# kartikmadhira1/YA_VO

Measured on AMD Instinct MI355X. Metric: frames/sec (detect+describe+match+PnP) on 1241×376 KITTI stereo; RMSE vs CPU ref, higher is better.
Workload: dtype u8

## Files before the change

ya_vo_amd/csrc/yavo_kernels.hip:

```cpp
#include <hip/hip_runtime.h>
#include <stdint.h>
#include <stdlib.h>
#include <string.h>

#include <algorithm>

#include "yavo_xlane.h"
#include "yavo_internal.h"


namespace yavo {

__device__ __forceinline__ int lane_id() { return (int)(threadIdx.x & 63); }

__device__ __forceinline__ int wave_incl_scan(int v) {
    v += __builtin_amdgcn_update_dpp(0, v, 0x111, 0xf, 0xf, false);
    v += __builtin_amdgcn_update_dpp(0, v, 0x112, 0xf, 0xf, false);
    v += __builtin_amdgcn_update_dpp(0, v, 0x114, 0xf, 0xf, false);
    v += __builtin_amdgcn_update_dpp(0, v, 0x118, 0xf, 0xf, false);
    v += __builtin_amdgcn_update_dpp(0, v, 0x142, 0xa, 0xf, false);
    v += __builtin_amdgcn_update_dpp(0, v, 0x143, 0xc, 0xf, false);
    return v;
}

// ... 929 lines not shown
                const int g = item & 3, kd = (item >> 2) * 64 + ln;
                const int k = (kd & 31) * G + (kd >> 5);
                const bool act = (kd >> 5) < G && k < nb;
                const uint32_t e = s_list[act ? k : nb - 1];
                const int i = (int)(e >> 16), row = r0 + (int)(e & 31u), col = (int)((e >> 5) & 2047u);
                const int id = (act && g == 0) ? src[i].z : 0;
                const int la = (row - rb) * LS + col;
                const int2* lo = loff + 64 * g;
                uint32_t w[2] = {0u, 0u};
#pragma unroll 1
                for (int c = 7; c >= 0; --c) {
                    const int2* oc = lo + 8 * c;
                    uint32_t acc = w[c >> 2];
#pragma unroll
                    for (int j = 7; j >= 0; --j) {
                        const int2 o = oc[j];
                        const uint32_t p1 = s_band[la + o.x], p2 = s_band[la + o.y];
                        acc = __builtin_amdgcn_alignbit(acc, p2 - p1, 31);
                    }
                    if (c >= 4) w[1] = acc;
                    else w[0] = acc;
                }
                if (act) {
                    reinterpret_cast<uint2*>(d_base + i)[g] = make_uint2(w[0], w[1]);
                    uint8_t* r = rec_b + (int64_t)i * 48;
                    if (g == 0) {
                        reinterpret_cast<int32_t*>(r)[0] = row;
                        reinterpret_cast<int32_t*>(r)[1] = col;
                        reinterpret_cast<int32_t*>(r)[2] = id;
                        r[12] = 0;
                    }
                    r[13 + 8 * g] = (uint8_t)w[0];
                    *reinterpret_cast<uint16_t*>(r + 14 + 8 * g) = (uint16_t)(w[0] >> 8);
                    *reinterpret_cast<uint32_t*>(r + 16 + 8 * g) = (w[0] >> 24) | (w[1] << 8);
                    r[20 + 8 * g] = (uint8_t)(w[1] >> 24);
                    if (g == 3) {
                        r[45] = 0;
                        *reinterpret_cast<uint16_t*>(r + 46) = 0;
                    }
                }
                asm volatile("" ::"v"(id));
            }
        }
        BP_MARK(1);
        __builtin_amdgcn_fence(__ATOMIC_RELEASE, "workgroup", "local");
        __builtin_amdgcn_s_barrier();
        __builtin_amdgcn_fence(__ATOMIC_ACQUIRE, "workgroup", "local");
        lb = __builtin_amdgcn_readfirstlane(s_next[0]);
        klo = __builtin_amdgcn_readfirstlane(s_next[1]);
        nbk = __builtin_amdgcn_readfirstlane(s_next[2]);
        BP_MARK(2);
    }
    BP_STORE();
}

__global__ void brief_loff_kernel(const int8_t* __restrict__ offsets, int LS, int2* __restrict__ loff) {
    const int t = threadIdx.x;
    const int8_t* o = offsets + 4 * t;
    loff[t] = make_int2((int)o[0] * LS + (int)o[1], (int)o[2] * LS + (int)o[3]);
}

void launch_brief(const uint8_t* blur, int n_images, int H, int W, const int8_t* offsets, const int32_t* kp_src,
                  const int32_t* kp_band, const int32_t* band_off, int max_kp, yv_keypoint* keypoints, Desc* desc,
                  int32_t* loff, bool new_loff, int32_t* heads, int max_workers, hipStream_t s) {
    const int total = ((H + BR_BAND - 1) / BR_BAND) * n_images;
    dim3 grid(std::max(1, std::min(max_workers, total)));
    const size_t lds = brief_lds_bytes(W);
    int2* lo = reinterpret_cast<int2*>(loff);
    if (new_loff) hipLaunchKernelGGL(brief_loff_kernel, dim3(1), dim3(256), 0, s, offsets, brief_lds_stride(W), lo);
    hipLaunchKernelGGL(brief_kernel, grid, dim3(BR_NT), lds, s, blur, H, W, kp_src, kp_band, band_off, max_kp,
                       keypoints, desc, lo, heads, total);
}

__global__ void pack_desc_kernel(const yv_keypoint* __restrict__ keypoints, const int32_t* __restrict__ kp_count,
                                 int max_kp, Desc* __restrict__ desc) {
    const int slot = blockIdx.y;
    const int i = blockIdx.x * blockDim.x + threadIdx.x;
    if (i >= kp_count[slot] || i >= max_kp) return;
    const uint8_t* rec = reinterpret_cast<const uint8_t*>(keypoints + (int64_t)slot * max_kp + i);
    Desc d;
#pragma unroll
    for (int q = 0; q < 8; ++q) {
        d.w[q] = (uint32_t)rec[13 + 4 * q] | ((uint32_t)rec[14 + 4 * q] << 8) | ((uint32_t)rec[15 + 4 * q] << 16) |
                 ((uint32_t)rec[16 + 4 * q] << 24);
    }
    desc[(int64_t)slot * max_kp + i] = d;
}

void launch_pack_desc(const yv_keypoint* keypoints, const int32_t* kp_count, int n_slots, int max_kp, Desc* desc,
                      hipStream_t s) {
    dim3 grid((max_kp + 255) / 256, n_slots);
    hipLaunchKernelGGL(pack_desc_kernel, grid, dim3(256), 0, s, keypoints, kp_count, max_kp, desc);
}

typedef int mm_v4i __attribute__((ext_vector_type(4)));
constexpr int MM_QT = 8;
constexpr int MM_QB = 4 * MM_QT * 16;
constexpr int MM_TC = 128;
constexpr int MM_ROW = 17;

__device__ __forceinline__ uint32_t expand_pm1(uint32_t nib) {
    const uint32_t spread = (nib * 0x00204081u) & 0x01010101u;
    return ~(spread * 0xFEu);
}

__device__ __forceinline__ uint4 expand16_pm1(uint32_t bits) {
    return make_uint4(expand_pm1(bits & 0xF), expand_pm1((bits >> 4) & 0xF), expand_pm1((bits >> 8) & 0xF),
                      expand_pm1((bits >> 12) & 0xF));
}

__device__ __forceinline__ int desc_popcount(const Desc& d) {
    int c = 0;
#pragma unroll
    for (int w = 0; w < 8; ++w) c += __popc(d.w[w]);
    return c;
}

__device__ __forceinline__ void top2_push2_i32(int& m1, int& m2, int x, int y) {
    const int hi = max(x, y), lo = min(x, y);
    m2 = max(min(m1, hi), max(m2, lo));
    m1 = max(m1, hi);
}

__device__ __forceinline__ void top2_merge_i32(int& m1, int& m2, int o1, int o2) {
    m2 = max(min(m1, o1), max(m2, o2));
    m1 = max(m1, o1);
}

__device__ __forceinline__ uint32_t mm_decode_key(int v) {
    const int dot = v >> 16;
    const uint32_t d = (uint32_t)((256 - dot) >> 1);
    const uint32_t jj = 0xFFFFu - ((uint32_t)v & 0xFFFFu);
    return (d << 16) | jj;
}

template <bool TOP2>
__device__ __forceinline__ void match_body(const Desc* __restrict__ desc, const int32_t* __restrict__ kp_count,
                                           const int32_t* __restrict__ pairs, int max_kp,
                                           uint32_t* __restrict__ match_key, uint32_t* __restrict__ match_key2) {
    __shared__ uint4 s_t[2][MM_TC * MM_ROW];
    const int pair = blockIdx.y;
    const int qi = pairs[2 * pair], ti = pairs[2 * pair + 1];
    const int nq = kp_count[qi], nt = kp_count[ti];
    const int q0 = blockIdx.x * MM_QB;
    if (q0 >= nq) return;
    const int tid = threadIdx.x, wave = tid >> 6, lane = tid & 63;
    const int col = lane & 15, g = lane >> 4;
    const Desc* qd = desc + (int64_t)qi * max_kp;
    const uint32_t* tw = reinterpret_cast<const uint32_t*>(desc + (int64_t)ti * max_kp);

    mm_v4i A[MM_QT][4];
#pragma unroll
    for (int qt = 0; qt < MM_QT; ++qt) {
        const int q = q0 + 16 * MM_QT * wave + 16 * qt + col;
        const Desc d = qd[q < nq ? q : 0];
#pragma unroll
        for (int s = 0; s < 4; ++s) {
            const uint32_t hi_mask = 0u - (uint32_t)(g >> 1);
            const uint32_t w = d.w[2 * s] ^ ((d.w[2 * s] ^ d.w[2 * s + 1]) & hi_mask);
            const uint32_t bits = (w >> (16 * (g & 1))) & 0xFFFFu;
            const uint4 e = expand16_pm1(bits);
            A[qt][s] = mm_v4i{(int)e.x, (int)e.y, (int)e.z, (int)e.w};
        }
    }
    int best[MM_QT][4];
#pragma unroll
    for (int qt = 0; qt < MM_QT; ++qt)
#pragma unroll
        for (int r = 0; r < 4; ++r) best[qt][r] = INT_MIN;
    int best2[TOP2 ? MM_QT : 1][4];
    if constexpr (TOP2) {
#pragma unroll
        for (int qt = 0; qt < MM_QT; ++qt)
#pragma unroll
            for (int r = 0; r < 4; ++r) best2[qt][r] = INT_MIN;
    }

    constexpr int kF = MM_TC * 16 / 256;
    uint32_t pre[kF];
    auto fetch = [&](int t0) {
#pragma unroll
        for (int k = 0; k < kF; ++k) {
            const int idx = tid + 256 * k, tt = idx >> 4, u = idx & 15;
            const int t = t0 + tt;
            pre[k] = t < nt ? tw[(int64_t)t * 8 + (u >> 1)] : 0u;
        }
    };
    auto store = [&](int buf) {
#pragma unroll
        for (int k = 0; k < kF; ++k) {
            const int idx = tid + 256 * k, tt = idx >> 4, u = idx & 15;
            const uint32_t bits = (pre[k] >> (16 * (u & 1))) & 0xFFFFu;
            s_t[buf][tt * MM_ROW + u] = expand16_pm1(bits);
        }
    };
    if (nt > 0) {
        fetch(0);
        store(0);
    }
    int buf = 0;
    for (int t0 = 0; t0 < nt; t0 += MM_TC) {
        const bool more = t0 + MM_TC < nt;
        if (more) fetch(t0 + MM_TC);
        __syncthreads();
#pragma unroll
        for (int tt0 = 0; tt0 < MM_TC; tt0 += 32) {
            if (t0 + tt0 >= nt) break;
            mm_v4i Ba[4], Bb[4];
#pragma unroll
            for (int s = 0; s < 4; ++s) {
                const uint4 va = s_t[buf][(tt0 + col) * MM_ROW + 4 * s + g];
                const uint4 vb = s_t[buf][(tt0 + 16 + col) * MM_ROW + 4 * s + g];
                Ba[s] = mm_v4i{(int)va.x, (int)va.y, (int)va.z, (int)va.w};
                Bb[s] = mm_v4i{(int)vb.x, (int)vb.y, (int)vb.z, (int)vb.w};
            }
            const int ja = t0 + tt0 + col, jb = ja + 16;
            {
                const int bias_a = ja < nt ? 0xFFFF - ja : -(1 << 30);
                const int bias_b = jb < nt ? 0xFFFF - jb : -(1 << 30);
#pragma unroll
                for (int qt = 0; qt < MM_QT; qt += 2) {
                    mm_v4i a0 = {0, 0, 0, 0}, b0 = {0, 0, 0, 0}, a1 = {0, 0, 0, 0}, b1 = {0, 0, 0, 0};
#pragma unroll
                    for (int s = 0; s < 4; ++s) {
                        a0 = __builtin_amdgcn_mfma_i32_16x16x64_i8(A[qt][s], Ba[s], a0, 0, 0, 0);
                        b0 = __builtin_amdgcn_mfma_i32_16x16x64_i8(A[qt][s], Bb[s], b0, 0, 0, 0);
                        a1 = __builtin_amdgcn_mfma_i32_16x16x64_i8(A[qt + 1][s], Ba[s], a1, 0, 0, 0);
                        b1 = __builtin_amdgcn_mfma_i32_16x16x64_i8(A[qt + 1][s], Bb[s], b1, 0, 0, 0);
                    }
#pragma unroll
                    for (int r = 0; r < 4; ++r) {
                        if constexpr (TOP2) {
                            top2_push2_i32(best[qt][r], best2[qt][r], (int)(((uint32_t)a0[r] << 16) + (uint32_t)bias_a),
                                           (int)(((uint32_t)b0[r] << 16) + (uint32_t)bias_b));
                            top2_push2_i32(best[qt + 1][r], best2[qt + 1][r],
                                           (int)(((uint32_t)a1[r] << 16) + (uint32_t)bias_a),
                                           (int)(((uint32_t)b1[r] << 16) + (uint32_t)bias_b));
                            continue;
                        }
                        best[qt][r] = max(best[qt][r], max((int)(((uint32_t)a0[r] << 16) + (uint32_t)bias_a),
                                                           (int)(((uint32_t)b0[r] << 16) + (uint32_t)bias_b)));
                        best[qt + 1][r] = max(best[qt + 1][r],
                                              max((int)(((uint32_t)a1[r] << 16) + (uint32_t)bias_a),
                                                  (int)(((uint32_t)b1[r] << 16) + (uint32_t)bias_b)));
                    }
                }
            }
        }
        if (more) {
            store(buf ^ 1);
            buf ^= 1;
        }
    }
#pragma unroll
    for (int qt = 0; qt < MM_QT; ++qt) {
#pragma unroll
        for (int r = 0; r < 4; ++r) {
            int v = best[qt][r];
            const int q = q0 + 16 * MM_QT * wave + 16 * qt + 4 * g + r;
            if constexpr (TOP2) {
                int v2 = best2[qt][r];
                top2_merge_i32(v, v2, xl::xor_row_i32<8>(v), xl::xor_row_i32<8>(v2));
                top2_merge_i32(v, v2, xl::xor_row_i32<4>(v), xl::xor_row_i32<4>(v2));
                top2_merge_i32(v, v2, xl::xor_row_i32<2>(v), xl::xor_row_i32<2>(v2));
                top2_merge_i32(v, v2, xl::xor_row_i32<1>(v), xl::xor_row_i32<1>(v2));
                if (col == r && q < nq) {
                    match_key[(int64_t)pair * max_kp + q] = v > -(1 << 29) ? mm_decode_key(v) : 0xFFFFFFFFu;
                    match_key2[(int64_t)pair * max_kp + q] = v2 > -(1 << 29) ? mm_decode_key(v2) : 0xFFFFFFFFu;
                }
                continue;
            }
            v = max(v, xl::xor_row_i32<8>(v));
            v = max(v, xl::xor_row_i32<4>(v));
            v = max(v, xl::xor_row_i32<2>(v));
            v = max(v, xl::xor_row_i32<1>(v));
            if (col == r && q < nq) {
                uint32_t key = 0xFFFFFFFFu;
                if (v != INT_MIN) {
                    const int dot = v >> 16;
                    const uint32_t d = (uint32_t)((256 - dot) >> 1);
                    const uint32_t jj = 0xFFFFu - ((uint32_t)v & 0xFFFFu);
                    key = (d << 16) | jj;
                }
                match_key[(int64_t)pair * max_kp + q] = key;
            }
        }
    }
}

__global__ __launch_bounds__(256) void match_kernel(const Desc* __restrict__ desc, const int32_t* __restrict__ kp_count,
                                                    const int32_t* __restrict__ pairs, int max_kp,
                                                    uint32_t* __restrict__ match_key) {
    match_body<false>(desc, kp_count, pairs, max_kp, match_key, nullptr);
}

__global__ __launch_bounds__(256) void match_top2_kernel(const Desc* __restrict__ desc,
                                                         const int32_t* __restrict__ kp_count,
                                                         const int32_t* __restrict__ pairs, int max_kp,
                                                         uint32_t* __restrict__ match_key,
                                                         uint32_t* __restrict__ match_key2) {
    match_body<true>(desc, kp_count, pairs, max_kp, match_key, match_key2);
}

constexpr int MF_TC = 128;
constexpr int MF_ROW = 9;
constexpr int MF2_QT = 4, MF2_WPE = 3;

__device__ __forceinline__ uint4 expand32_fp4(uint32_t w) {
    constexpr uint32_t kBit1 = 0x22222222u;
    return make_uint4((w << 1) & kBit1, w & kBit1, (w >> 1) & kBit1, (w >> 2) & kBit1);
}

typedef int mf_v8i __attribute__((ext_vector_type(8)));
typedef float mf_v16f __attribute__((ext_vector_type(16)));

__device__ __forceinline__ mf_v16f mfma_fp4_32(const mm_v4i& a, const mm_v4i& b, const mf_v16f& c) {
    const mf_v8i a8 = __builtin_shufflevector(a, a, 0, 1, 2, 3, -1, -1, -1, -1);
    const mf_v8i b8 = __builtin_shufflevector(b, b, 0, 1, 2, 3, -1, -1, -1, -1);
    return __builtin_amdgcn_mfma_scale_f32_32x32x64_f8f6f4(a8, b8, c, 4, 4, 0, 133, 0, 133);
}

__device__ __forceinline__ uint32_t max16_u32(uint32_t best, const mf_v16f& a) {
    auto u = [&](int i) { return __float_as_uint(a[i]); };
    const uint32_t m0 = max(u(0), max(u(1), u(2))), m1 = max(u(3), max(u(4), u(5)));
    const uint32_t m2 = max(u(6), max(u(7), u(8))), m3 = max(u(9), max(u(10), u(11)));
    const uint32_t m4 = max(u(12), max(u(13), u(14)));
    const uint32_t m5 = max(m0, max(m1, m2)), m6 = max(m3, max(m4, u(15)));
    return max(best, max(m5, m6));
}

__device__ __forceinline__ uint32_t umed3_pos(uint32_t a, uint32_t b, uint32_t c) {
    return __float_as_uint(__builtin_amdgcn_fmed3f(__uint_as_float(a), __uint_as_float(b), __uint_as_float(c)));
}

__device__ __forceinline__ void top2_merge3(uint32_t h0, uint32_t l0, uint32_t h1, uint32_t l1, uint32_t h2,
                                            uint32_t l2, uint32_t& m1, uint32_t& m2) {
    m1 = max(h0, max(h1, h2));
    m2 = max(umed3_pos(h0, h1, h2), max(l0, max(l1, l2)));
}

__device__ __forceinline__ void top2_16_u32(uint32_t& m1, uint32_t& m2, const mf_v16f& a) {
    auto u = [&](int i) { return __float_as_uint(a[i]); };
    uint32_t h[5], l[5];
#pragma unroll
    for (int k = 0; k < 5; ++k) {
        h[k] = max(u(3 * k), max(u(3 * k + 1), u(3 * k + 2)));
        l[k] = umed3_pos(u(3 * k), u(3 * k + 1), u(3 * k + 2));
    }
    uint32_t a1, a2, b1, b2;
    top2_merge3(h[0], l[0], h[1], l[1], h[2], l[2], a1, a2);
    top2_merge3(h[3], l[3], h[4], l[4], u(15), 0u, b1, b2);
    top2_merge3(a1, a2, b1, b2, m1, m2, m1, m2);
}

__device__ __forceinline__ uint32_t fp4_decode_key(uint32_t bits, int pa) {
    const int iv = (int)__uint_as_float(bits) - (1 << 21);
    const uint32_t d = (uint32_t)(pa - (iv >> 11));
    const uint32_t jj = 2047u - ((uint32_t)iv & 2047u);
    return (d << 16) | jj;
}

template <int QT, int WPE, bool TOP2>
__global__ __launch_bounds__(256) __attribute__((amdgpu_waves_per_eu(WPE, 8))) void match_fp4_kernel(
    const Desc* __restrict__ desc, const int32_t* __restrict__ kp_count, const int32_t* __restrict__ pairs, int max_kp,
    uint32_t* __restrict__ match_key, uint32_t* __restrict__ match_key2) {
    constexpr int QB = 4 * QT * 32;
    __shared__ uint4 s_t[2][MF_TC * MF_ROW];
    __shared__ float s_c[2][MF_TC];
    const int pair = blockIdx.y;
    const int qi = pairs[2 * pair], ti = pairs[2 * pair + 1];
    const int nq = kp_count[qi], nt = kp_count[ti];
    const int q0 = blockIdx.x * QB;
    if (q0 >= nq) return;
    const int tid = threadIdx.x, wave = tid >> 6, lane = tid & 63;
    const int n = lane & 31, h = lane >> 5;
    const uint32_t* qw = reinterpret_cast<const uint32_t*>(desc + (int64_t)qi * max_kp);
    const uint32_t* tw = reinterpret_cast<const uint32_t*>(desc + (int64_t)ti * max_kp);

    mm_v4i B[QT][4];
    uint32_t raw[QT][4];
#pragma unroll
    for (int qt = 0; qt < QT; ++qt) {
        const int q = q0 + 32 * QT * wave + 32 * qt + n;
        const uint32_t* w = qw + (int64_t)(q < nq ? q : 0) * 8 + h;
#pragma unroll
        for (int s = 0; s < 4; ++s) raw[qt][s] = w[2 * s];
    }
#pragma unroll
    for (int qt = 0; qt < QT; ++qt)
#pragma unroll
        for (int s = 0; s < 4; ++s) {
            const uint4 e = expand32_fp4(raw[qt][s]);
            B[qt][s] = mm_v4i{(int)e.x, (int)e.y, (int)e.z, (int)e.w};
        }
    uint32_t best[QT];
#pragma unroll
    for (int qt = 0; qt < QT; ++qt) best[qt] = 0u;
    uint32_t best2[TOP2 ? QT : 1];
    if constexpr (TOP2) {
#pragma unroll
        for (int qt = 0; qt < QT; ++qt) best2[qt] = 0u;
    }

    constexpr int kF = MF_TC * 8 / 256;
    uint32_t pre[kF];
    auto fetch = [&](int t0) {
#pragma unroll
        for (int k = 0; k < kF; ++k) {
            const int idx = tid + 256 * k, tt = idx >> 3, u = idx & 7;
            const int t = t0 + tt;
            pre[k] = t < nt ? tw[(int64_t)t * 8 + u] : 0u;
        }
    };
    auto store = [&](int buf, int t0) {
#pragma unroll
        for (int k = 0; k < kF; ++k) {
            const int idx = tid + 256 * k, tt = idx >> 3, u = idx & 7;
            s_t[buf][tt * MF_ROW + u] = expand32_fp4(pre[k]);
            uint32_t pc = __builtin_popcount(pre[k]);
            pc += xl::dpp<0xB1>(pc);
            pc += xl::dpp<0x4E>(pc);
            pc += xl::dpp<0x141>(pc);
            const int t = t0 + tt;
            if (u == 0) s_c[buf][tt] = t < nt ? (float)((2047 - t) - 2048 * (int)pc + (1 << 21)) : 0.f;
        }
    };
    if (nt > 0) {
        fetch(0);
        store(0, 0);
    }
    int buf = 0;
    for (int t0 = 0; t0 < nt; t0 += MF_TC) {
        const bool more = t0 + MF_TC < nt;
        if (more) fetch(t0 + MF_TC);
        __syncthreads();
#pragma unroll
        for (int tt0 = 0; tt0 < MF_TC; tt0 += 32) {
            if (t0 + tt0 >= nt) break;
            mm_v4i A[4];
#pragma unroll
            for (int s = 0; s < 4; ++s) {
                const uint4 v = s_t[buf][(tt0 + n) * MF_ROW + 2 * s + h];
                A[s] = mm_v4i{(int)v.x, (int)v.y, (int)v.z, (int)v.w};
            }
            mf_v16f C;
#pragma unroll
            for (int k = 0; k < 4; ++k) {
                const float4 c4 = *reinterpret_cast<const float4*>(&s_c[buf][tt0 + 8 * k + 4 * h]);
                C[4 * k] = c4.x;
                C[4 * k + 1] = c4.y;
                C[4 * k + 2] = c4.z;
                C[4 * k + 3] = c4.w;
            }
#pragma unroll
            for (int qt = 0; qt < QT; qt += 2) {
                mf_v16f a0 = mfma_fp4_32(A[0], B[qt][0], C);
                mf_v16f a1 = mfma_fp4_32(A[0], B[qt + 1][0], C);
#pragma unroll
                for (int s = 1; s < 4; ++s) {
                    a0 = mfma_fp4_32(A[s], B[qt][s], a0);
                    a1 = mfma_fp4_32(A[s], B[qt + 1][s], a1);
                }
                if constexpr (TOP2) {
                    top2_16_u32(best[qt], best2[qt], a0);
                    top2_16_u32(best[qt + 1], best2[qt + 1], a1);
                } else {
                    best[qt] = max16_u32(best[qt], a0);
                    best[qt + 1] = max16_u32(best[qt + 1], a1);
                }
            }
        }
        if (more) {
            store(buf ^ 1, t0 + MF_TC);
            buf ^= 1;
        }
    }
#pragma unroll
    for (int qt = 0; qt < QT; ++qt) {
        uint32_t v = best[qt];
        uint32_t v2 = 0u;
        if constexpr (TOP2) {
            const uint32_t o1 = (uint32_t)__shfl_xor((int)v, 32, 64), o2 = (uint32_t)__shfl_xor((int)best2[qt], 32, 64);
            v2 = max(min(v, o1), max(best2[qt], o2));
            v = max(v, o1);
        } else {
            v = max(v, (uint32_t)__shfl_xor((int)v, 32, 64));
        }
        int pa = 0;
#pragma unroll
        for (int s = 0; s < 4; ++s)
#pragma unroll
            for (int r = 0; r < 4; ++r) pa += __popc((uint32_t)B[qt][s][r]);
        pa += __shfl_xor(pa, 32, 64);
        const int q = q0 + 32 * QT * wave + 32 * qt + n;
        if (h == 0 && q < nq) {
            uint32_t key = 0xFFFFFFFFu;
            if (nt > 0) {
                const int iv = (int)__uint_as_float(v) - (1 << 21);
                const uint32_t d = (uint32_t)(pa - (iv >> 11));
                const uint32_t jj = 2047u - ((uint32_t)iv & 2047u);
                key = (d << 16) | jj;
            }
            match_key[(int64_t)pair * max_kp + q] = key;
            if constexpr (TOP2) match_key2[(int64_t)pair * max_kp + q] = v2 != 0u ? fp4_decode_key(v2, pa) : 0xFFFFFFFFu;
        }
    }
}

namespace {
template <int QT, int WPE, bool TOP2>
void launch_fp4(const MatchLists& lists, const int32_t* pairs, int n_pairs, uint32_t* match_key, uint32_t* match_key2,
                hipStream_t s) {
    constexpr int QB = 4 * QT * 32;
    dim3 grid((lists.max_kp + QB - 1) / QB, n_pairs);
    hipLaunchKernelGGL((match_fp4_kernel<QT, WPE, TOP2>), grid, dim3(256), 0, s, lists.desc, lists.kp_count, pairs,
                       lists.max_kp, match_key, match_key2);
}
}

void launch_match(const MatchLists& lists, const int32_t* pairs, int n_pairs, int max_train, uint32_t* match_key,
                  uint32_t* match_key2, hipStream_t s) {
    if (max_train > 2048) {
        dim3 grid((lists.max_kp + MM_QB - 1) / MM_QB, n_pairs);
        if (match_key2)
            hipLaunchKernelGGL(match_top2_kernel, grid, dim3(256), 0, s, lists.desc, lists.kp_count, pairs,
                               lists.max_kp, match_key, match_key2);
        else
            hipLaunchKernelGGL(match_kernel, grid, dim3(256), 0, s, lists.desc, lists.kp_count, pairs, lists.max_kp,
                               match_key);
        return;
    }
    if (!match_key2) launch_fp4<4, 3, false>(lists, pairs, n_pairs, match_key, nullptr, s);
    else launch_fp4<MF2_QT, MF2_WPE, true>(lists, pairs, n_pairs, match_key, match_key2, s);
}

constexpr int FZ_NT = 1024;
constexpr int REC_DW = 25;

__device__ __forceinline__ int block_min_int(int v, int* s_tmp) {
    for (int off = 32; off > 0; off >>= 1) v = min(v, __shfl_xor(v, off, 64));
    const int wave = (int)threadIdx.x >> 6;
    if (lane_id() == 0) s_tmp[wave] = v;
    __syncthreads();
    int r = s_tmp[0];
    for (int w = 1; w < (int)(blockDim.x >> 6); ++w) r = min(r, s_tmp[w]);
    __syncthreads();
    return r;
}

__device__ __forceinline__ int outlier_limit(int min_d, int thr) {
    const int twice = (int)((uint32_t)min_d * 2u);
    return twice > thr ? twice : thr;
}

template <bool ROBUST>
__global__ __launch_bounds__(FZ_NT) void match_finalize_kernel(
    uint32_t* __restrict__ match_key, const yv_keypoint* __restrict__ keypoints,
    const int32_t* __restrict__ kp_count, const int32_t* __restrict__ pairs, int max_kp, int thr,
    yv_match* __restrict__ matches, int32_t* __restrict__ match_count, yv_match* __restrict__ filtered,
    int32_t* __restrict__ filt_count, int2* __restrict__ match_dj, int32_t* __restrict__ match_lim,
    int32_t* __restrict__ kp_count_copy, int n_slots, FinalizeRobust rb) {
    __shared__ int s_dist[kMaxKp];
    if (kp_count_copy && blockIdx.x == 0)
        for (int i = (int)threadIdx.x; i < n_slots; i += FZ_NT) kp_count_copy[i] = kp_count[i];
    __shared__ int s_j[kMaxKp];
    __shared__ int s_pos[kMaxKp];
    __shared__ int s_tmp[40];
    const int pair = blockIdx.x;
    const int tid = threadIdx.x;
    const int qi = pairs[2 * pair], ti = pairs[2 * pair + 1];
    const int nq = kp_count[qi];
    uint32_t* keys = match_key + (int64_t)pair * max_kp;
    int local_min = 0x7fffffff;
    for (int i = tid; i < nq; i += FZ_NT) {
        const uint32_t k = keys[i];
        keys[i] = 0xFFFFFFFFu;
        const int d = (k == 0xFFFFFFFFu) ? 0x7fffffff : (int)(k >> 16);
        s_dist[i] = d;
        s_j[i] = (k == 0xFFFFFFFFu) ? -1 : (int)(k & 0xFFFFu);
        local_min = min(local_min, d);
        if constexpr (ROBUST) {
            uint32_t* keys2 = rb.match_key2 + (int64_t)pair * max_kp;
            const uint32_t k2 = keys2[i];
            keys2[i] = 0xFFFFFFFFu;
            const int j1 = s_j[i];
            const int d2 = (k2 == 0xFFFFFFFFu) ? 0x7fffffff : (int)(k2 >> 16);
            const int j2 = (k2 == 0xFFFFFFFFu) ? -1 : (int)(k2 & 0xFFFFu);
            rb.nn2[(int64_t)pair * max_kp + i] = make_int4(d, j1, d2, j2);
            bool ok = true;
            if (rb.flags & kMatchRatio) ok = (int64_t)d * rb.den < (int64_t)d2 * rb.num;
            if (rb.flags & kMatchMutual) {
                const uint32_t rk = j1 >= 0 ? rb.rev_key[(int64_t)pair * max_kp + j1] : 0xFFFFFFFFu;
                ok = ok && rk != 0xFFFFFFFFu && (int)(rk & 0xFFFFu) == i;
            }
            s_pos[i] = ok ? 1 : 0;
        }
    }
    const int min_d = block_min_int(local_min, s_tmp);
    const int lim = outlier_limit(min_d, thr);
    if constexpr (ROBUST) {
        const int nt = kp_count[ti];
        uint32_t* rkeys = rb.rev_key + (int64_t)pair * max_kp;
        for (int j = tid; j < nt; j += FZ_NT) {
            const uint32_t rk = rkeys[j];
            rkeys[j] = 0xFFFFFFFFu;
            rb.rev[(int64_t)pair * max_kp + j] = (rk == 0xFFFFFFFFu) ? -1 : (int)(rk & 0xFFFFu);
        }
    }
    int flags[4], cnt = 0;
    int2* dj = match_dj + (int64_t)pair * max_kp;
#pragma unroll
    for (int u = 0; u < 4; ++u) {
        const int i = tid * 4 + u;
        flags[u] = (i < nq && s_dist[i] < lim) ? 1 : 0;
        if constexpr (ROBUST) {
            if (i < nq) {
                flags[u] &= s_pos[i];
                rb.keep[(int64_t)pair * max_kp + i] = (uint8_t)flags[u];
            }
        }
        cnt += flags[u];
        if (i < nq) dj[i] = make_int2(s_dist[i], s_j[i]);
    }
    int total = 0;
    int off = block_excl_scan<FZ_NT>(cnt, s_tmp, &total);
#pragma unroll
    for (int u = 0; u < 4; ++u) {
        const int i = tid * 4 + u;
        if (i < nq) s_pos[i] = flags[u] ? off : -1;
        off += flags[u];
    }
    __syncthreads();
    const uint32_t* qrec = reinterpret_cast<const uint32_t*>(keypoints + (int64_t)qi * max_kp);
    const uint32_t* trec = reinterpret_cast<const uint32_t*>(keypoints + (int64_t)ti * max_kp);
    uint32_t* out_all = reinterpret_cast<uint32_t*>(matches + (int64_t)pair * max_kp);
    uint32_t* out_f = reinterpret_cast<uint32_t*>(filtered + (int64_t)pair * max_kp);
    const int ndw = nq * REC_DW;
    constexpr int FZ_U = 4;
    for (int dw0 = tid; dw0 < ndw; dw0 += FZ_U * FZ_NT) {
        uint32_t v[FZ_U];
        int ii[FZ_U], ff[FZ_U];
#pragma unroll
        for (int u = 0; u < FZ_U; ++u) {
            const int dw = min(dw0 + u * FZ_NT, ndw - 1);
            const int i = dw / REC_DW, f = dw - i * REC_DW;
            const int j = s_j[i];
            const uint32_t* src = f < 12 ? qrec + (int64_t)i * 12 + f : trec + (int64_t)max(j, 0) * 12 + min(f - 12, 2);
            v[u] = *src;
            ii[u] = i;
            ff[u] = f;
        }
#pragma unroll
        for (int u = 0; u < FZ_U; ++u) {
            const int dw = dw0 + u * FZ_NT;
            if (dw >= ndw) break;
            const int i = ii[u], f = ff[u];
            uint32_t x = v[u];
            if (f == 11) x &= 0xFFu;
            else if (f >= 12 && (f >= 15 || s_j[i] < 0)) x = 0;
            if (f == 24) x = (uint32_t)s_dist[i];
            out_all[dw] = x;
            const int p = s_pos[i];
            if (p >= 0) {
                if (f == 3 || f == 15) x = (x & ~0xFFu) | 1u;
                out_f[(int64_t)p * REC_DW + f] = x;
            }
        }
    }
    if (tid == 0) {
        match_count[pair] = nq;
        filt_count[pair] = total;
        match_lim[pair] = lim;
    }
}

void launch_match_finalize(uint32_t* match_key, const MatchLists& lists, const int32_t* pairs, int n_pairs, int thr,
                           const MatchRecords& out, const FinalizeRobust* rb, hipStream_t s, int32_t* kp_count_copy,
                           int n_slots) {
    const auto kernel = !rb ? match_finalize_kernel<false> : match_finalize_kernel<true>;
    hipLaunchKernelGGL(kernel, dim3(n_pairs), dim3(FZ_NT), 0, s, match_key, lists.keypoints, lists.kp_count, pairs,
                       lists.max_kp, thr, out.matches, out.match_count, out.filtered, out.filt_count, out.match_dj,
                       out.match_lim, kp_count_copy, n_slots, rb ? *rb : FinalizeRobust{});
}

__global__ __launch_bounds__(FZ_NT) void filter_records_kernel(const yv_match* __restrict__ in, int n, int thr,
                                                               yv_match* __restrict__ out,
                                                               int32_t* __restrict__ out_count) {
    __shared__ int s_pos[kMaxKp];
    __shared__ int s_tmp[40];
    const int tid = threadIdx.x;
    const uint32_t* src = reinterpret_cast<const uint32_t*>(in);
    int local_min = 0x7fffffff;
    for (int i = tid; i < n; i += FZ_NT) local_min = min(local_min, (int)src[(int64_t)i * REC_DW + 24]);
    const int min_d = block_min_int(local_min, s_tmp);
    const int lim = outlier_limit(min_d, thr);
    int flags[4], cnt = 0;
#pragma unroll
    for (int u = 0; u < 4; ++u) {
        const int i = tid * 4 + u;
        flags[u] = (i < n && (int)src[(int64_t)i * REC_DW + 24] < lim) ? 1 : 0;
        cnt += flags[u];
    }
    int total = 0;
    int off = block_excl_scan<FZ_NT>(cnt, s_tmp, &total);
#pragma unroll
    for (int u = 0; u < 4; ++u) {
        const int i = tid * 4 + u;
        if (i < n) s_pos[i] = flags[u] ? off : -1;
        off += flags[u];
    }
    __syncthreads();
    uint32_t* dst = reinterpret_cast<uint32_t*>(out);
    for (int dw = tid; dw < n * REC_DW; dw += FZ_NT) {
        const int i = dw / REC_DW;
        const int f = dw - i * REC_DW;
        const int p = s_pos[i];
        if (p < 0) continue;
        uint32_t v = src[dw];
        if (f == 3 || f == 15) v = (v & ~0xFFu) | 1u;
        dst[(int64_t)p * REC_DW + f] = v;
    }
    if (tid == 0) *out_count = total;
}

void launch_filter_records(const yv_match* in, int n, int thr, yv_match* out, int32_t* out_count, hipStream_t s) {
    hipLaunchKernelGGL(filter_records_kernel, dim3(1), dim3(FZ_NT), 0, s, in, n, thr, out, out_count);
}

}

#ifdef YAVO_LM_PROFILE
extern "C" int yv_debug_brief_prof(unsigned long long* out ) {
    return hipMemcpyFromSymbol(out, HIP_SYMBOL(yavo::g_brief_prof), sizeof(unsigned long long) * 16384 * 6) ==
                   hipSuccess ? 0 : -2;
}
extern "C" int yv_debug_det_prof(unsigned long long* out ) {
    return hipMemcpyFromSymbol(out, HIP_SYMBOL(yavo::g_det_prof), sizeof(unsigned long long) * 131072 * 6) ==
                   hipSuccess ? 0 : -2;
}
#endif

namespace yavo {
__global__ void xlane_check_kernel(int32_t* out) {
    const int l = threadIdx.x;
    out[0 * 64 + l] = xl::xor_row_i32<1>(l);
    out[1 * 64 + l] = xl::xor_row_i32<2>(l);
    out[2 * 64 + l] = xl::xor_row_i32<4>(l);
    out[3 * 64 + l] = xl::xor_row_i32<8>(l);
    uint32_t a = (uint32_t)l, b = 100u + (uint32_t)l;
    xl::swap_halves<16>(a, b);
    out[4 * 64 + l] = (int32_t)a;
    out[5 * 64 + l] = (int32_t)b;
    a = (uint32_t)l;
    b = 100u + (uint32_t)l;
    xl::swap_halves<32>(a, b);
    out[6 * 64 + l] = (int32_t)a;
    out[7 * 64 + l] = (int32_t)b;
}
}

extern "C" int yv_debug_xlane(int32_t* d_out , void* stream) {
    if (!d_out) return -1;
    hipLaunchKernelGGL(yavo::xlane_check_kernel, dim3(1), dim3(64), 0, reinterpret_cast<hipStream_t>(stream), d_out);
    return hipGetLastError() == hipSuccess ? 0 : -2;
}
```

Baseline: 255,200.

## Stream train descriptors per-wave into registers instead of block-shared LDS tiles

The fp4 MFMA matcher no longer stages 128-row train tiles in shared memory behind block-wide barriers. Each wave now loads its own 32-row train slice straight into registers, expands it there, and prefetches two tiles ahead, leaving only a small per-wave LDS slot for the bias vector, guarded by wave barriers. It also flattens the grid to 1D with an XCD swizzle and makes waves skip query tiles beyond nq. In exchange every wave refetches the train descriptors from global memory or cache, and register pressure rises.

```diff
diff --git a/ya_vo_amd/csrc/yavo_kernels.hip b/ya_vo_amd/csrc/yavo_kernels.hip
--- a/ya_vo_amd/csrc/yavo_kernels.hip
+++ b/ya_vo_amd/csrc/yavo_kernels.hip
@@ -1255,8 +1255,6 @@
     match_body<true>(desc, kp_count, pairs, max_kp, match_key, match_key2);
 }
 
-constexpr int MF_TC = 128;
-constexpr int MF_ROW = 9;
 constexpr int MF2_QT = 4, MF2_WPE = 3;
 
 __device__ __forceinline__ uint4 expand32_fp4(uint32_t w) {
@@ -1317,35 +1315,40 @@
 __global__ __launch_bounds__(256) __attribute__((amdgpu_waves_per_eu(WPE, 8))) void match_fp4_kernel(
     const Desc* __restrict__ desc, const int32_t* __restrict__ kp_count, const int32_t* __restrict__ pairs, int max_kp,
     uint32_t* __restrict__ match_key, uint32_t* __restrict__ match_key2) {
+    static_assert(QT % 2 == 0, "query tiles run in pairs");
     constexpr int QB = 4 * QT * 32;
-    __shared__ uint4 s_t[2][MF_TC * MF_ROW];
-    __shared__ float s_c[2][MF_TC];
-    const int pair = blockIdx.y;
+    __shared__ float s_c[4][2][32];
+    const int nqb = (max_kp + QB - 1) / QB;
+    const int lb = xcd_swizzle((int)blockIdx.x, (int)gridDim.x);
+    const int pair = lb / nqb;
     const int qi = pairs[2 * pair], ti = pairs[2 * pair + 1];
     const int nq = kp_count[qi], nt = kp_count[ti];
-    const int q0 = blockIdx.x * QB;
+    const int q0 = (lb - pair * nqb) * QB;
     if (q0 >= nq) return;
-    const int tid = threadIdx.x, wave = tid >> 6, lane = tid & 63;
+    const int tid = threadIdx.x, wave = __builtin_amdgcn_readfirstlane(tid >> 6), lane = tid & 63;
     const int n = lane & 31, h = lane >> 5;
-    const uint32_t* qw = reinterpret_cast<const uint32_t*>(desc + (int64_t)qi * max_kp);
-    const uint32_t* tw = reinterpret_cast<const uint32_t*>(desc + (int64_t)ti * max_kp);
+    const int qw0 = q0 + 32 * QT * wave;
+    const int nqt = min((nq - qw0 + 31) >> 5, QT);
+    if (nqt <= 0) return;
+    const uint4* qv = reinterpret_cast<const uint4*>(desc + (int64_t)qi * max_kp);
+    const uint4* tv = reinterpret_cast<const uint4*>(desc + (int64_t)ti * max_kp);
 
     mm_v4i B[QT][4];
-    uint32_t raw[QT][4];
+    uint4 raw[QT];
 #pragma unroll
     for (int qt = 0; qt < QT; ++qt) {
-        const int q = q0 + 32 * QT * wave + 32 * qt + n;
-        const uint32_t* w = qw + (int64_t)(q < nq ? q : 0) * 8 + h;
-#pragma unroll
-        for (int s = 0; s < 4; ++s) raw[qt][s] = w[2 * s];
-    }
-#pragma unroll
-    for (int qt = 0; qt < QT; ++qt)
+        const int q = qw0 + 32 * qt + n;
+        raw[qt] = qv[(int64_t)(q < nq ? q : 0) * 2 + h];
+    }
+#pragma unroll
+    for (int qt = 0; qt < QT; ++qt) {
+        const uint32_t w[4] = {raw[qt].x, raw[qt].y, raw[qt].z, raw[qt].w};
 #pragma unroll
         for (int s = 0; s < 4; ++s) {
-            const uint4 e = expand32_fp4(raw[qt][s]);
+            const uint4 e = expand32_fp4(w[s]);
             B[qt][s] = mm_v4i{(int)e.x, (int)e.y, (int)e.z, (int)e.w};
         }
+    }
     uint32_t best[QT];
 #pragma unroll
     for (int qt = 0; qt < QT; ++qt) best[qt] = 0u;
@@ -1355,78 +1358,71 @@
         for (int qt = 0; qt < QT; ++qt) best2[qt] = 0u;
     }
 
-    constexpr int kF = MF_TC * 8 / 256;
-    uint32_t pre[kF];
     auto fetch = [&](int t0) {
-#pragma unroll
-        for (int k = 0; k < kF; ++k) {
-            const int idx = tid + 256 * k, tt = idx >> 3, u = idx & 7;
-            const int t = t0 + tt;
-            pre[k] = t < nt ? tw[(int64_t)t * 8 + u] : 0u;
-        }
+        const int t = t0 + n;
+        return tv[(int64_t)(t < nt ? t : 0) * 2 + h];
     };
-    auto store = [&](int buf, int t0) {
-#pragma unroll
-        for (int k = 0; k < kF; ++k) {
-            const int idx = tid + 256 * k, tt = idx >> 3, u = idx & 7;
-            s_t[buf][tt * MF_ROW + u] = expand32_fp4(pre[k]);
-            uint32_t pc = __builtin_popcount(pre[k]);
-            pc += xl::dpp<0xB1>(pc);
-            pc += xl::dpp<0x4E>(pc);
-            pc += xl::dpp<0x141>(pc);
-            const int t = t0 + tt;
-            if (u == 0) s_c[buf][tt] = t < nt ? (float)((2047 - t) - 2048 * (int)pc + (1 << 21)) : 0.f;
+    auto prep = [&](const uint4& raw, int t0, int slot, mm_v4i (&A)[4]) {
+        const int t = t0 + n;
+        const uint32_t m = t < nt ? 0xFFFFFFFFu : 0u;
+        const uint32_t w[4] = {raw.x & m, raw.y & m, raw.z & m, raw.w & m};
+        uint32_t pc = __popc(w[0]) + __popc(w[1]) + __popc(w[2]) + __popc(w[3]), po = pc;
+        xl::swap_halves<32>(pc, po);
+        pc += po;
+        if (h == 0) s_c[wave][slot][n] = t < nt ? (float)((2047 - t) - 2048 * (int)pc + (1 << 21)) : 0.f;
+#pragma unroll
+        for (int s = 0; s < 4; ++s) {
+            const uint4 e = expand32_fp4(w[s]);
+            A[s] = mm_v4i{(int)e.x, (int)e.y, (int)e.z, (int)e.w};
         }
     };
-    if (nt > 0) {
-        fetch(0);
-        store(0, 0);
-    }
+    auto read_c = [&](int slot) {
+        __builtin_amdgcn_fence(__ATOMIC_RELEASE, "wavefront");
+        __builtin_amdgcn_wave_barrier();
+        __builtin_amdgcn_fence(__ATOMIC_ACQUIRE, "wavefront");
+        mf_v16f C;
+#pragma unroll
+        for (int k = 0; k < 4; ++k) {
+            const float4 c4 = *reinterpret_cast<const float4*>(&s_c[wave][slot][8 * k + 4 * h]);
+            C[4 * k] = c4.x;
+            C[4 * k + 1] = c4.y;
+            C[4 * k + 2] = c4.z;
+            C[4 * k + 3] = c4.w;
+        }
+        return C;
+    };
+    auto tile_pair = [&](int qt, const mm_v4i (&A)[4], const mf_v16f& C) {
+        if (qt >= nqt) return;
+        mf_v16f a0 = mfma_fp4_32(A[0], B[qt][0], C);
+        mf_v16f a1 = mfma_fp4_32(A[0], B[qt + 1][0], C);
+#pragma unroll
+        for (int s = 1; s < 4; ++s) {
+            a0 = mfma_fp4_32(A[s], B[qt][s], a0);
+            a1 = mfma_fp4_32(A[s], B[qt + 1][s], a1);
+        }
+        if constexpr (TOP2) {
+            top2_16_u32(best[qt], best2[qt], a0);
+            top2_16_u32(best[qt + 1], best2[qt + 1], a1);
+        } else {
+            best[qt] = max16_u32(best[qt], a0);
+            best[qt + 1] = max16_u32(best[qt + 1], a1);
+        }
+    };
+    mm_v4i A[4], An[4];
+    prep(fetch(0), 0, 0, A);
+    uint4 nxt = fetch(32);
     int buf = 0;
-    for (int t0 = 0; t0 < nt; t0 += MF_TC) {
-        const bool more = t0 + MF_TC < nt;
-        if (more) fetch(t0 + MF_TC);
-        __syncthreads();
-#pragma unroll
-        for (int tt0 = 0; tt0 < MF_TC; tt0 += 32) {
-            if (t0 + tt0 >= nt) break;
-            mm_v4i A[4];
-#pragma unroll
-            for (int s = 0; s < 4; ++s) {
-                const uint4 v = s_t[buf][(tt0 + n) * MF_ROW + 2 * s + h];
-                A[s] = mm_v4i{(int)v.x, (int)v.y, (int)v.z, (int)v.w};
-            }
-            mf_v16f C;
-#pragma unroll
-            for (int k = 0; k < 4; ++k) {
-                const float4 c4 = *reinterpret_cast<const float4*>(&s_c[buf][tt0 + 8 * k + 4 * h]);
-                C[4 * k] = c4.x;
-                C[4 * k + 1] = c4.y;
-                C[4 * k + 2] = c4.z;
-                C[4 * k + 3] = c4.w;
-            }
-#pragma unroll
-            for (int qt = 0; qt < QT; qt += 2) {
-                mf_v16f a0 = mfma_fp4_32(A[0], B[qt][0], C);
-                mf_v16f a1 = mfma_fp4_32(A[0], B[qt + 1][0], C);
-#pragma unroll
-                for (int s = 1; s < 4; ++s) {
-                    a0 = mfma_fp4_32(A[s], B[qt][s], a0);
-                    a1 = mfma_fp4_32(A[s], B[qt + 1][s], a1);
-                }
-                if constexpr (TOP2) {
-                    top2_16_u32(best[qt], best2[qt], a0);
-                    top2_16_u32(best[qt + 1], best2[qt + 1], a1);
-                } else {
-                    best[qt] = max16_u32(best[qt], a0);
-                    best[qt + 1] = max16_u32(best[qt + 1], a1);
-                }
-            }
-        }
-        if (more) {
-            store(buf ^ 1, t0 + MF_TC);
-            buf ^= 1;
-        }
+    for (int t0 = 0; t0 < nt; t0 += 32) {
+        const uint4 nn = fetch(t0 + 64);
+        const mf_v16f C = read_c(buf);
+        tile_pair(0, A, C);
+        prep(nxt, t0 + 32, buf ^ 1, An);
+#pragma unroll
+        for (int qt = 2; qt < QT; qt += 2) tile_pair(qt, A, C);
+#pragma unroll
+        for (int s = 0; s < 4; ++s) A[s] = An[s];
+        nxt = nn;
+        buf ^= 1;
     }
 #pragma unroll
     for (int qt = 0; qt < QT; ++qt) {
@@ -1465,7 +1461,7 @@
 void launch_fp4(const MatchLists& lists, const int32_t* pairs, int n_pairs, uint32_t* match_key, uint32_t* match_key2,
                 hipStream_t s) {
     constexpr int QB = 4 * QT * 32;
-    dim3 grid((lists.max_kp + QB - 1) / QB, n_pairs);
+    dim3 grid((unsigned)(((lists.max_kp + QB - 1) / QB) * n_pairs));
     hipLaunchKernelGGL((match_fp4_kernel<QT, WPE, TOP2>), grid, dim3(256), 0, s, lists.desc, lists.kp_count, pairs,
                        lists.max_kp, match_key, match_key2);
 }
```

Result: no change. 255,800, median of 2 (+0.2%).
